# thygate/stable-diffusion-webui-depthmap-script

Measured on AMD Instinct MI355X. Metric: depth+stereo pairs/sec @1024x1024, higher is better.
Workload: dtype f16 (network) / f64 (stereo, normal map); 1 GPU; BASELINE config c3: MiDaS 3.1 DPT BEiT-L/16 512 forward (fp16, random-init weights seed 0, net 512x512, 1025 tokens) + depth->u16 + create_stereoimages(polylines_sharp, left-right, divergence 2.5%) + create_normalmap (Sobel 3) on 32 x 1024x1024 RGB per GPU, inputs resident in HBM; depth_network=dpt_beit_large_512, height=1024, width=1024, forward_launch=eager, library_convolutions=MIOpen, heuristic solver choice, overlap=single stream, parallelism=units sharded over 1 GPU(s), no data-path collective

## Files before the change

### include/depthstereo.h

```cpp
#ifndef DEPTHSTEREO_H
#define DEPTHSTEREO_H

#include <stddef.h>
#include <stdint.h>

#ifdef __cplusplus
extern "C" {
#endif

#define DS_VERSION 100

#define DS_OK            0
#define DS_EINVAL       -1
#define DS_EUNSUPPORTED -2
#define DS_EHIP         -3
#define DS_ENOMEM       -4

#define DS_DEPTH_U16 0
#define DS_DEPTH_F32 1
#define DS_DEPTH_F64 2

#define DS_FILL_NONE                0
#define DS_FILL_NAIVE               1
#define DS_FILL_NAIVE_INTERPOLATING 2
// ... 102 lines not shown
#define DS_PIX_U8  0
#define DS_PIX_U16 1
#define DS_PIX_I32 2
#define DS_PIX_F32 3

int ds_resize_lanczos(ds_ctx *ctx, const void *src, int pix, int n, int in_h, int in_w, int64_t src_px_stride, int64_t src_row_stride,
                      int64_t src_img_stride, void *dst, int out_h, int out_w, const int32_t *h_bounds, const void *h_coeffs, int h_taps,
                      const int32_t *v_bounds, const void *v_coeffs, int v_taps, void *tmp, void *stream);

#define DS_CD_WIDEN       0
#define DS_CD_SINGLE_BAND 1
#define DS_CD_MULTI_BAND  2
#define DS_CD_WORKSPACE_BLOCKS 256
int ds_custom_depth_to_f64(ds_ctx *ctx, const void *src, int pix, int n, int h, int w, int64_t src_px_stride, int64_t src_row_stride,
                           int64_t src_img_stride, int rule, double *out, double *workspace, void *stream);

#define DS_DTYPE_F16  1
#define DS_DTYPE_BF16 2
#define DS_DTYPE_F32  3

int ds_attention_fwd(ds_ctx *ctx, const void *qk, const void *vt, const void *bias_packed, void *out,
                     int B, int Np, int H, int n_valid, float scale, int dtype, void *stream);

int ds_attention_bias_pack(ds_ctx *ctx, const float *bias, int H, int n, int Np, int dtype, void *packed, void *stream);

int ds_attention_reload_env(void);

int ds_preprocess_bicubic(ds_ctx *ctx, const void *images, void *out, int batch, int in_h, int in_w, int out_h, int out_w,
                          int flip_channels, const float *mean, const float *std, int dtype, void *stream);

int ds_residual_layernorm(ds_ctx *ctx, const void *x, const void *branch, const void *gamma, const void *ln_weight,
                          const void *ln_bias, void *x_out, void *h_out, int64_t rows, int channels, float eps, int dtype,
                          void *stream);

int ds_reassemble_readout(ds_ctx *ctx, const void *proj, const void *clsvec, void *out, int batch, int tokens, int channels,
                          int dtype, void *stream);

int ds_bias_act_nhwc(ds_ctx *ctx, const void *x, const void *bias, const void *res1, const void *res2, void *out,
                     int64_t elements, int channels, int relu, int dtype, void *stream);

int ds_group_norm_nchw(ds_ctx *ctx, const void *x, const void *gamma, const void *beta, const void *res, void *out, int n, int channels,
                       int hw, int groups, float eps, int relu, int dtype, void *stream);

int ds_linear(ds_ctx *ctx, const void *x, const void *w, const void *bias, void *y, int64_t rows, int64_t out_features,
              int64_t in_features, int64_t ldy, int act, int dtype, void *stream);

int ds_linear_residual(ds_ctx *ctx, const void *x, const void *w, const void *bias, const void *gamma, const void *res, void *y,
                       int64_t rows, int64_t out_features, int64_t in_features, int dtype, void *stream);

int ds_linear_vt(ds_ctx *ctx, const void *w_v, const void *h, void *vt, int64_t channels, int64_t batch, int64_t tokens,
                 int64_t in_features, int dtype, void *stream);

int ds_linear_qkv(ds_ctx *ctx, const void *h, const void *w_qk, const void *b_qk, const void *w_v, void *qk, void *vt,
                  int64_t batch, int64_t tokens, int64_t qk_features, int64_t v_channels, int64_t in_features, int dtype, void *stream);

int ds_linear_shuffle(ds_ctx *ctx, const void *x, const void *w, const void *bias, void *y, int64_t pixels, int64_t in_features,
                      int width, int stride, int out_channels, int dtype, void *stream);

int ds_linear_readout(ds_ctx *ctx, const void *x, const void *w_tok, const void *cls_vec, void *y, int64_t images,
                      int64_t tokens_padded, int64_t tokens, int64_t out_features, int64_t in_features, int dtype, void *stream);

int ds_conv3x3_nhwc_pair(ds_ctx *ctx, const void *x0, const void *w0, void *y0, int batch0, int height0, int width0,
                         const void *x1, const void *w1, void *y1, int batch1, int height1, int width1,
                         int in_channels, int out_channels, int dtype, void *stream);

typedef struct ds_rows_problem {
    const void *x;
    int64_t x_row_pitch;
    const void *w;
    const void *bias;
    void *y;
} ds_rows_problem;
int ds_linear_rows4(ds_ctx *ctx, const ds_rows_problem *problems, int count, int64_t rows, int64_t out_features,
                    int64_t in_features, int dtype, void *stream);

int ds_row_stats(ds_ctx *ctx, const void *x, void *stats, int64_t rows, int channels, float eps, int dtype, void *stream);
int ds_linear_ln(ds_ctx *ctx, const void *x, const void *w_scaled, const float *colsum, const void *bias, const void *stats, void *y,
                 int64_t rows, int64_t out_features, int64_t in_features, int64_t ldy, int act, int dtype, void *stream);
int ds_linear_vt_ln(ds_ctx *ctx, const void *w_v_scaled, const float *colsum, const void *x, const void *stats, void *vt,
                    int64_t channels, int64_t batch, int64_t tokens, int64_t in_features, int dtype, void *stream);

int ds_linear_reload_env(void);

int ds_conv3x3_nhwc(ds_ctx *ctx, const void *x, const void *w, const void *bias, const void *res1, const void *res2, void *y,
                    int batch, int height, int width, int in_channels, int out_channels, int act, int dtype, void *stream);

int ds_conv3x3_nhwc_circular(ds_ctx *ctx, const void *x, const void *w, const void *bias, const void *res1, const void *res2, void *y,
                             int batch, int height, int width, int in_channels, int out_channels, int act, int dtype, void *stream);

int ds_upsample_bilinear_nhwc(ds_ctx *ctx, const void *in, void *out, int batch, int channels, int in_h, int in_w,
                              int out_h, int out_w, int align_corners, int dtype, void *stream);

int ds_dpt_head_front(ds_ctx *ctx, const void *x, const void *w, const void *bias, void *out, int batch, int in_h, int in_w,
                      int out_h, int out_w, int in_channels, int out_channels, int dtype, void *stream);

int ds_dpt_head_tail(ds_ctx *ctx, const void *x, int batch, int in_h, int in_w, int out_h, int out_w,
                     const void *conv3_wfrag, const float *conv3_bias, const float *conv1_weight, float conv1_bias,
                     int relu_out, void *out, int dtype, void *stream);

int ds_dpt_head_tail_circular(ds_ctx *ctx, const void *x, int batch, int in_h, int in_w, int out_h, int out_w,
                              const void *conv3_wfrag, const float *conv3_bias, const float *conv1_weight, float conv1_bias,
                              int relu_out, void *out, int dtype, void *stream);

int ds_gconv3x3_nhwc_f32(ds_ctx *ctx, const float *x, const float *w_gtio, const float *bias, float *y, int batch, int height, int width,
                         int channels, int channels_per_group, int relu, void *stream);
int ds_add_relu_f32(ds_ctx *ctx, const float *a, const float *b, float *y, int64_t count, void *stream);

int ds_bias_act_f32(ds_ctx *ctx, const float *x, const float *bias, const float *res, float *y, int64_t pixels, int channels, int relu,
                    void *stream);

int ds_dwconv_nhwc(ds_ctx *ctx, const void *x, const float *w, const float *bias_in, const float *bias, void *y, int batch, int in_h,
                   int in_w, int channels, int out_h, int out_w, int kernel, int stride, int pad_top, int pad_left, int dtype, void *stream);
int ds_relu_cat_f32(ds_ctx *ctx, const float *a, const float *b, float *y, int batch, int64_t plane, int channels_a, int channels_b, int layout,
                    void *stream);

int ds_boost_blend(ds_ctx *ctx, float *dst, int64_t dst_row_stride, int height, int width, const void *patches,
                   int n_patches, const float *preds, int pred_size, const float *mask_template, int mask_size,
                   void *stream);

int ds_preprocess_bicubic_rows(ds_ctx *ctx, const void *images, void *rows, int batch, int in_h, int in_w, int out_h, int out_w,
                               int flip_channels, const float *mean, const float *std, int patch, int n_pad, int kpad, int dtype,
                               void *stream);

int ds_tokens_fixup(ds_ctx *ctx, void *tokens, const void *cls, int batch, int n_pad, int n_valid, int channels, int dtype, void *stream);

int ds_upsample_bicubic_to_f32(ds_ctx *ctx, const void *in, void *out, int batch, int in_h, int in_w, int out_h, int out_w, int dtype,
                               void *stream);

int ds_im2col3x3_s2_nhwc(ds_ctx *ctx, const void *x, void *rows, int batch, int height, int width, int channels, int circular, int dtype,
                         void *stream);

#ifdef __cplusplus
}
#endif
#endif
```

### stable-diffusion-webui-depthmap-script_amd/csrc/ds_linear.hip

```cpp
#include "ds_common.h"

#include <stdlib.h>
#include <atomic>
#include <type_traits>

typedef _Float16 lf16x8 __attribute__((ext_vector_type(8)));
typedef __bf16 lbf16x8 __attribute__((ext_vector_type(8)));
typedef _Float16 lf16x4 __attribute__((ext_vector_type(4)));
typedef __bf16 lbf16x4 __attribute__((ext_vector_type(4)));
typedef float lf32x16 __attribute__((ext_vector_type(16)));
typedef float lf32x4 __attribute__((ext_vector_type(4)));

#if defined(DS_EXPERIMENTS) && defined(DS_LIN_MFMA32)
#define LN_MF16 0
#else
#define LN_MF16 1
#endif

#define LN_THREADS 512
#define LN_LDS_BYTES 131072
#define LN_HALF 16384
#define LN_B_BASE 65536

template <int BF16> struct ln_traits;
// ... 1087 lines not shown
    const int row0 = 32 * rb, col0 = cbk * 64, rows = P.rows;
    const int K = P.K, nst = K >> 7;
    const unsigned rowbytes = (unsigned)K * (unsigned)sizeof(T);
    const unsigned pitch = (unsigned)pk->pitch[prob];
    unsigned srcA, srcB[2];
    {
        const int j = 8 * (wid & 3) + (lane >> 3);
        const int jr = min(row0 + j, rows - 1) - row0;
        srcA = (unsigned)jr * pitch + (unsigned)(((lane & 7) ^ ((j >> 1) & 7)) << 4) + (unsigned)(wid >> 2) * 128u;
    }
#pragma unroll
    for (int i = 0; i < 2; ++i) {
        const int j = 8 * ((2 * wid + i) & 7) + (lane >> 3);
        srcB[i] = (unsigned)j * rowbytes + (unsigned)(((lane & 7) ^ ((j >> 1) & 7)) << 4) + (unsigned)(wid >> 2) * 128u;
    }
    const unsigned char *xb = (const unsigned char *)pk->x[prob] + (size_t)row0 * pitch;
    const unsigned char *wb = (const unsigned char *)pk->w[prob] + (size_t)col0 * rowbytes;
    const unsigned lds0 = (unsigned)(size_t)(__attribute__((address_space(3))) void *)lds;
    const bool mw = wid < 2;
    unsigned offA[8], offB[8];
#pragma unroll
    for (int u = 0; u < 8; ++u) {
        const int j = u >> 2, ks = u & 3;
        const unsigned sl = (unsigned)((LN_MF16 ? 4 * (ks >> 1) + (lane >> 4) : 2 * ks + hi) ^ ((lane >> 1) & 7)) << 4;
        const int lrow = LN_MF16 ? 16 * (ks & 1) + (lane & 15) : l31;
        offA[u] = (unsigned)j * 4096u + (unsigned)lrow * 128u + sl;
        offB[u] = 8192u + (unsigned)j * 8192u + (unsigned)((wid & 1) * 32 + lrow) * 128u + sl;
    }
    LN_SMALL_ACC(mine);
    const int e_row = row0 + LN_SMALL_ROW;
    const int e_cb = col0 + (wid & 1) * 32 + LN_SMALL_COL;
    const T *bias = (const T *)pk->bias[prob];
    V8 e_bv[2];
    if (mw && bias) {
#pragma unroll
        for (int k = 0; k < 2; ++k) e_bv[k] = *(const V8 *)(bias + e_cb + LN_SMALL_DCOL(k));
    }
#pragma unroll
    for (int t = 0; t < S - 1; ++t) TH_STAGE(t);
    V8 fa0[8], fb0[8], fa1[8], fb1[8];
    LN_WAIT_VM(12);
    LN_BARRIER();
    if (mw) {
        TH_READ(fa0, fb0, 0);
        __builtin_amdgcn_sched_barrier(0);
        LN_WAIT_LGKM0();
        __builtin_amdgcn_sched_barrier(0);
    }
    int st = 0;
    for (; st + 1 < nst; st += 2) {
        TH_STEP(fa0, fb0, fa1, fb1, st);
        TH_STEP(fa1, fb1, fa0, fb0, st + 1);
    }
    if (st < nst) TH_STEP(fa0, fb0, fa1, fb1, st);
    LN_WAIT_VM(0);
    if (!mw) return;

    T *yb = (T *)pk->y[prob];
#pragma unroll
    for (int k = 0; k < 2; ++k) {
        const int row = e_row + LN_SMALL_DROW(k), col = e_cb + LN_SMALL_DCOL(k);
        V8 bv;
        if (bias) bv = e_bv[k];
        else {
#pragma unroll
            for (int t = 0; t < 8; ++t) bv[t] = (T)0.f;
        }
        float v[8];
        LN_SMALL_V(v, mine, k);
        V8 o;
#pragma unroll
        for (int t = 0; t < 8; t += 2) {
            const lf32x2 u = {v[t] + (float)bv[t], v[t + 1] + (float)bv[t + 1]};
            o[t] = (T)u[0];
            o[t + 1] = (T)u[1];
        }
        if (row < rows) *(V8 *)(yb + (size_t)row * P.N + col) = o;
    }
}
#undef TH_STEP
#undef TH_READ
#undef TH_STAGE

struct LinOptions { int early, grid, ragged, ragged_den, ragged_ring, ragged_ksplit, ragged_ksplit_min, ragged_ksplit_keep, ragged_pipe, ragged_thin; };
static LinOptions g_lin_options;
static std::atomic<int> g_lin_options_state{0};
static void ln_read_options()
{
    auto geti = [](const char *name, int dflt) { const char *e = getenv(name); return e ? atoi(e) : dflt; };
    LinOptions o;
    o.early = geti("DS_LIN_EARLY", 1);
    o.grid = geti("DS_LIN_GRID", 0);
    o.ragged = geti("DS_LIN_RAGGED", 1);
    o.ragged_den = geti("DS_LIN_RAGGED_DEN", 4);
    o.ragged_ring = geti("DS_LIN_RAGGED_RING", 0);
    o.ragged_ksplit = geti("DS_LIN_RAGGED_KSPLIT", 1);
    o.ragged_ksplit_min = geti("DS_LIN_RAGGED_KSPLIT_MIN", 32);
    o.ragged_ksplit_keep = geti("DS_LIN_RAGGED_KSPLIT_KEEP", 8);
    if (o.ragged_ksplit_keep < 1) o.ragged_ksplit_keep = 1;
    o.ragged_pipe = geti("DS_LIN_RAGGED_PIPE", 1);
    o.ragged_thin = geti("DS_LIN_RAGGED_THIN", 1);
    g_lin_options = o;
    g_lin_options_state.store(1, std::memory_order_release);
}
static const LinOptions &ln_options()
{
    if (!g_lin_options_state.load(std::memory_order_acquire)) ln_read_options();
    return g_lin_options;
}
DS_API int ds_linear_reload_env(void)
{
    ln_read_options();
    return DS_OK;
}

#define LN_RG_COUNTER_BYTES 4096
#define LN_RG_MAX_WG 1024
static int ln_ragged_workspace(ds_ctx *ctx, int grid, hipStream_t stream)
{
    if (grid > LN_RG_MAX_WG) return 1;
    if (ctx->lin_ws && ctx->lin_ws_cleared == ctx->lin_ws) return DS_OK;
    hipStreamCaptureStatus cap = hipStreamCaptureStatusNone;
    if (hipStreamIsCapturing(stream, &cap) != hipSuccess || cap != hipStreamCaptureStatusNone) { (void)hipGetLastError(); return 1; }
    if (!ctx->lin_ws) {
        const int rc = ds_ctx_reserve(ctx, &ctx->lin_ws, &ctx->lin_ws_bytes, LN_RG_COUNTER_BYTES + (size_t)LN_RG_MAX_WG * 32768);
        if (rc != DS_OK) return rc;
    }
    DS_HIP_CHECK(hipMemsetAsync(ctx->lin_ws, 0, LN_RG_COUNTER_BYTES, stream));
    DS_HIP_CHECK(hipStreamSynchronize(stream));
    ctx->lin_ws_cleared = ctx->lin_ws;
    return DS_OK;
}

static int ln_ksplit_arch_ok(ds_ctx *ctx)
{
    static std::atomic<uint64_t> checked{0}, ok{0};
    const uint64_t bit = 1ull << (ctx->device & 63);
    if (!(checked.load(std::memory_order_acquire) & bit)) {
        hipDeviceProp_t prop;
        bool good = false;
        if (hipGetDeviceProperties(&prop, ctx->device) == hipSuccess)
            good = strncmp(prop.gcnArchName, "gfx950", 6) == 0 || strncmp(prop.gcnArchName, "gfx942", 6) == 0;
        else (void)hipGetLastError();
        if (good) ok.fetch_or(bit, std::memory_order_relaxed);
        checked.fetch_or(bit, std::memory_order_release);
    }
    return (ok.load(std::memory_order_relaxed) & bit) != 0;
}

template <int BF16, int EPI, int CONV, int RES, int VT = 0, int NH = 0>
static int ln_launch(ds_ctx *ctx, const LinParams &P0, hipStream_t stream)
{
    static std::atomic<uint64_t> attr_done{0};
    auto fn = k_linear256<BF16, EPI, CONV, RES, VT, NH>;
    DS_HIP_CHECK(hipSetDevice(ctx->device));
    const uint64_t bit = 1ull << (ctx->device & 63);
    if (!(attr_done.load(std::memory_order_relaxed) & bit)) {
        DS_HIP_CHECK(hipFuncSetAttribute((const void *)fn, hipFuncAttributeMaxDynamicSharedMemorySize, LN_LDS_BYTES));
        if constexpr (CONV == 0) {
            DS_HIP_CHECK(hipFuncSetAttribute((const void *)k_linear_ragged<BF16, EPI, RES, VT, 3>, hipFuncAttributeMaxDynamicSharedMemorySize, 3 * RG_SLOT));
            DS_HIP_CHECK(hipFuncSetAttribute((const void *)k_linear_ragged<BF16, EPI, RES, VT, 6>, hipFuncAttributeMaxDynamicSharedMemorySize, 6 * RG_SLOT));
            DS_HIP_CHECK(hipFuncSetAttribute((const void *)k_linear_ragged<BF16, EPI, RES, VT, 6, 1>, hipFuncAttributeMaxDynamicSharedMemorySize, 6 * RG_SLOT));
            if constexpr (VT == 0 && RES <= 1)
                DS_HIP_CHECK(hipFuncSetAttribute((const void *)k_linear_thin<BF16, EPI, RES>, hipFuncAttributeMaxDynamicSharedMemorySize, 6 * RG_SLOT));
        }
        attr_done.fetch_or(bit, std::memory_order_relaxed);
    }
    if (!ctx->ncu) {
        int ncu = 0;
        DS_HIP_CHECK(hipDeviceGetAttribute(&ncu, hipDeviceAttributeMultiprocessorCount, ctx->device));
        ctx->ncu = ncu >= 8 ? ncu / 8 * 8 : 8;
    }
    const LinOptions &O = ln_options();
    int grid = ctx->ncu;
    if (O.grid >= 8) grid = O.grid / 8 * 8;
    LinParams P = P0;
    P.bnw = NH ? 128 : 256;
    P.early = O.early;
#ifdef DS_EXPERIMENTS
    if (P.ablate) P.early = 0;
#endif
    const int ntiles = P.nbm * P.nbn;
    int ragged = 0;
    if (CONV == 0 && ntiles > grid) {
        const int r = ntiles % grid;
        if (O.ragged && r > 0 && O.ragged_den > 0 && O.ragged_den * r <= grid) ragged = r;
    }
    P.n_main = ntiles - ragged;
    const int deep = O.ragged_ring ? O.ragged_ring == 6 : 8 * ragged <= grid;
    bool thin = false;
    int th_nrb = 0;
    if constexpr (CONV == 0 && VT == 0 && RES <= 1) {
        th_nrb = (P.M - (P.nbm - 1) * 256 + 31) / 32;
        thin = O.ragged_thin && ragged > 0 && ragged == P.nbn && P.nbm >= 2 && (P.nbm - 1) % 8 == 0 && P.K % 128 == 0 && P.N % 64 == 0 &&
               O.ragged_ksplit <= 1 && th_nrb * (P.N / 64) <= ctx->ncu;
    }
    P.th_nrb = th_nrb;
    int ksl = 0;
    if (CONV == 0 && ragged && !thin && deep && 8 * ragged * (int)sizeof(int) <= LN_RG_COUNTER_BYTES && ln_ksplit_arch_ok(ctx)) {
        const int nt = P.K / 64;
        while (nt >= O.ragged_ksplit_min && (2 << ksl) <= O.ragged_ksplit && 8 * ragged * (2 << ksl) <= grid && nt % (2 << ksl) == 0 &&
               nt / (2 << ksl) >= O.ragged_ksplit_keep) ++ksl;
    }
    if (ksl > 0) {
        const int rc = ln_ragged_workspace(ctx, grid, stream);
        if (rc == DS_OK) { P.rg_cnt = (int *)ctx->lin_ws; P.rg_ws = (float *)((char *)ctx->lin_ws + LN_RG_COUNTER_BYTES); }
        else if (rc == 1) ksl = 0;
        else return rc;
    }
    P.rg_ksl = ksl;
    const int kt0 = ds_kt_begin(ctx, P.kt_kind, stream);
    hipLaunchKernelGGL(fn, dim3(P.n_main < grid ? P.n_main : grid), dim3(LN_THREADS), LN_LDS_BYTES, stream, P);
    ds_kt_end(ctx, P.kt_kind, kt0, stream);
    if constexpr (CONV == 0) {
        const int kt1 = ragged ? ds_kt_begin(ctx, P.kt_kind + DS_KT_RAGGED, stream) : -1;
        if (thin) {
            if constexpr (VT == 0 && RES <= 1) hipLaunchKernelGGL((k_linear_thin<BF16, EPI, RES>), dim3(th_nrb * (P.N / 64)), dim3(LN_THREADS), 6 * RG_SLOT, stream, P);
        } else if (ragged && deep && O.ragged_pipe) hipLaunchKernelGGL((k_linear_ragged<BF16, EPI, RES, VT, 6, 1>), dim3((8 * ragged) << ksl), dim3(LN_THREADS), 6 * RG_SLOT, stream, P);
        else if (ragged && deep) hipLaunchKernelGGL((k_linear_ragged<BF16, EPI, RES, VT, 6>), dim3((8 * ragged) << ksl), dim3(LN_THREADS), 6 * RG_SLOT, stream, P);
        else if (ragged) hipLaunchKernelGGL((k_linear_ragged<BF16, EPI, RES, VT, 3>), dim3(8 * ragged), dim3(LN_THREADS), 3 * RG_SLOT, stream, P);
        ds_kt_end(ctx, P.kt_kind + DS_KT_RAGGED, kt1, stream);
    }
    DS_HIP_CHECK(hipGetLastError());
    return DS_OK;
}

template <int BF16>
static int ln_launch_qkv(ds_ctx *ctx, const LinParams &PQ, const LinParams &PV0, hipStream_t stream)
{
    static std::atomic<uint64_t> attr_done{0};
    auto fn = k_linear256<BF16, 0, 0, 0, 4>;
    DS_HIP_CHECK(hipSetDevice(ctx->device));
    const uint64_t bit = 1ull << (ctx->device & 63);
    if (!(attr_done.load(std::memory_order_relaxed) & bit)) {
        DS_HIP_CHECK(hipFuncSetAttribute((const void *)fn, hipFuncAttributeMaxDynamicSharedMemorySize, LN_LDS_BYTES));
        DS_HIP_CHECK(hipFuncSetAttribute((const void *)k_linear_ragged<BF16, 0, 0, 1, 3>, hipFuncAttributeMaxDynamicSharedMemorySize, 3 * RG_SLOT));
        DS_HIP_CHECK(hipFuncSetAttribute((const void *)k_linear_ragged<BF16, 0, 0, 1, 6>, hipFuncAttributeMaxDynamicSharedMemorySize, 6 * RG_SLOT));
        DS_HIP_CHECK(hipFuncSetAttribute((const void *)k_linear_ragged<BF16, 0, 0, 1, 6, 1>, hipFuncAttributeMaxDynamicSharedMemorySize, 6 * RG_SLOT));
        attr_done.fetch_or(bit, std::memory_order_relaxed);
    }
    if (!ctx->ncu) {
        int ncu = 0;
        DS_HIP_CHECK(hipDeviceGetAttribute(&ncu, hipDeviceAttributeMultiprocessorCount, ctx->device));
        ctx->ncu = ncu >= 8 ? ncu / 8 * 8 : 8;
    }
    const LinOptions &O = ln_options();
    int grid = ctx->ncu;
    if (O.grid >= 8) grid = O.grid / 8 * 8;
    const int t0 = PQ.nbm * PQ.nbn, t1 = PV0.nbm * PV0.nbn, ntiles = t0 + t1;
    int ragged = 0;
    if (ntiles > grid) {
        const int r = ntiles % grid;
        if (O.ragged && r > 0 && O.ragged_den > 0 && O.ragged_den * r <= grid && r <= t1) ragged = r;
    }
    LinParams P = PQ, PV = PV0;
    P.bnw = PV.bnw = 256;
    P.early = O.early;
    P.x1 = PV.x; P.w1 = PV.w; P.y1 = PV.y;
    P.seg_t0 = t0; P.M1 = PV.M; P.nbm1 = PV.nbm; P.nbn1 = PV.nbn;
    P.vt_np = PV.vt_np; P.vt_c = PV.vt_c; P.vt_magic = PV.vt_magic;
    P.n_main = ntiles - ragged;
    PV.n_main = t1 - ragged;
    const int kt0 = ds_kt_begin(ctx, DS_KT_LINEAR, stream);
    hipLaunchKernelGGL(fn, dim3(P.n_main < grid ? P.n_main : grid), dim3(LN_THREADS), LN_LDS_BYTES, stream, P);
    ds_kt_end(ctx, DS_KT_LINEAR, kt0, stream);
    if (ragged) {
        const int deep = O.ragged_ring ? O.ragged_ring == 6 : 8 * ragged <= grid;
        const int kt1 = ds_kt_begin(ctx, DS_KT_LINEAR + DS_KT_RAGGED, stream);
        if (deep && O.ragged_pipe) hipLaunchKernelGGL((k_linear_ragged<BF16, 0, 0, 1, 6, 1>), dim3(8 * ragged), dim3(LN_THREADS), 6 * RG_SLOT, stream, PV);
        else if (deep) hipLaunchKernelGGL((k_linear_ragged<BF16, 0, 0, 1, 6>), dim3(8 * ragged), dim3(LN_THREADS), 6 * RG_SLOT, stream, PV);
        else hipLaunchKernelGGL((k_linear_ragged<BF16, 0, 0, 1, 3>), dim3(8 * ragged), dim3(LN_THREADS), 3 * RG_SLOT, stream, PV);
        ds_kt_end(ctx, DS_KT_LINEAR + DS_KT_RAGGED, kt1, stream);
    }
    DS_HIP_CHECK(hipGetLastError());
    return DS_OK;
}

template <int BF16>
static int ln_dispatch_dense(ds_ctx *ctx, const LinParams &P, int act, hipStream_t st)
{
    if (act == 1) return ln_launch<BF16, 1, 0, 0>(ctx, P, st);
    if (act == 2) return ln_launch<BF16, 2, 0, 0>(ctx, P, st);
    return ln_launch<BF16, 0, 0, 0>(ctx, P, st);
}

template <int BF16, int CIRC>
static int ln_dispatch_conv(ds_ctx *ctx, const LinParams &P, int act, hipStream_t st)
{
    constexpr int CV = CIRC ? 3 : 1, CVR = CIRC ? 4 : 2;
    const int res = P.res1 ? (P.res2 ? 2 : 1) : 0;
    if (act & 4) {
        if (P.N % 256 == 0 && (act & 3) == 2 && res == 0) return ln_launch<BF16, 2, CVR, 0>(ctx, P, st);
        ds_set_error("ds_conv3x3_nhwc[_circular]: act 4 (ReLU on x) is built for act 2 | 4 without residual operands and out_channels %% 256 == 0");
        return DS_EUNSUPPORTED;
    }
    if (P.N % 256 != 0) {
        if (act == 2) return ln_launch<BF16, 2, CV, 0, 0, 1>(ctx, P, st);
        return ln_launch<BF16, 0, CV, 0, 0, 1>(ctx, P, st);
    }
    if (act == 2) {
        if (res == 2) return ln_launch<BF16, 2, CV, 2>(ctx, P, st);
        if (res == 1) return ln_launch<BF16, 2, CV, 1>(ctx, P, st);
        return ln_launch<BF16, 2, CV, 0>(ctx, P, st);
    }
    if (res == 2) return ln_launch<BF16, 0, CV, 2>(ctx, P, st);
    if (res == 1) return ln_launch<BF16, 0, CV, 1>(ctx, P, st);
    return ln_launch<BF16, 0, CV, 0>(ctx, P, st);
}

DS_API int ds_linear(ds_ctx *ctx, const void *x, const void *w, const void *bias, void *y, int64_t rows, int64_t out_features,
                     int64_t in_features, int64_t ldy, int act, int dtype, void *stream)
{
    DS_REQUIRE(ctx && x && w && y, DS_EINVAL, "ds_linear: null argument");
    DS_REQUIRE(rows >= 256 && rows < (1ll << 31) - 256, DS_EINVAL, "ds_linear: rows must be >= 256 (one tile)");
    DS_REQUIRE(out_features > 0 && out_features % 256 == 0, DS_EINVAL, "ds_linear: out_features must be a multiple of 256");
    DS_REQUIRE(in_features >= 128 && in_features % 128 == 0 && in_features <= 16384, DS_EINVAL,
               "ds_linear: in_features must be a multiple of 128 (<= 16384)");
    DS_REQUIRE(ldy >= out_features && ldy % 8 == 0, DS_EINVAL, "ds_linear: ldy must be >= out_features and a multiple of 8");
    DS_REQUIRE(((uintptr_t)x & 15) == 0 && ((uintptr_t)w & 15) == 0 && ((uintptr_t)y & 15) == 0 && (!bias || ((uintptr_t)bias & 15) == 0), DS_EINVAL,
               "ds_linear: x, w (the LDS-DMA sources), y and bias must be 16-byte aligned");
    DS_REQUIRE(act >= 0 && act <= 2, DS_EINVAL, "ds_linear: act must be 0 (none), 1 (erf-GELU) or 2 (ReLU)");
    DS_REQUIRE(dtype == DS_DTYPE_F16 || dtype == DS_DTYPE_BF16, DS_EINVAL, "ds_linear: dtype must be f16 or bf16");
    LinParams P;
    memset(&P, 0, sizeof(P));
    P.x = x; P.w = w; P.bias = bias; P.y = y;
    P.M = (int)rows; P.N = (int)out_features; P.K = (int)in_features;
    P.nbm = (int)((rows + 255) / 256); P.nbn = (int)(out_features / 256);
    P.ldy = ldy;
    P.kt_kind = act == 1 ? DS_KT_LINEAR_GELU : DS_KT_LINEAR;
#ifdef DS_EXPERIMENTS
    P.ablate = getenv("DS_LIN_ABLATE") ? atoi(getenv("DS_LIN_ABLATE")) : 0;
    P.stagger = getenv("DS_LIN_STAGGER_US") ? (int)(atof(getenv("DS_LIN_STAGGER_US")) * 100.0) : 0;
#endif
    return dtype == DS_DTYPE_F16 ? ln_dispatch_dense<0>(ctx, P, act, (hipStream_t)stream) : ln_dispatch_dense<1>(ctx, P, act, (hipStream_t)stream);
}

DS_API int ds_linear_residual(ds_ctx *ctx, const void *x, const void *w, const void *bias, const void *gamma, const void *res, void *y,
                              int64_t rows, int64_t out_features, int64_t in_features, int dtype, void *stream)
{
    DS_REQUIRE(ctx && x && w && y && res, DS_EINVAL, "ds_linear_residual: null argument");
    DS_REQUIRE(rows >= 256 && rows < (1ll << 31) - 256, DS_EINVAL, "ds_linear_residual: rows must be >= 256 (one tile)");
    DS_REQUIRE(out_features > 0 && out_features % 256 == 0, DS_EINVAL, "ds_linear_residual: out_features must be a multiple of 256");
    DS_REQUIRE(in_features >= 128 && in_features % 128 == 0 && in_features <= 16384, DS_EINVAL,
               "ds_linear_residual: in_features must be a multiple of 128 (<= 16384)");
    DS_REQUIRE(dtype == DS_DTYPE_F16 || dtype == DS_DTYPE_BF16, DS_EINVAL, "ds_linear_residual: dtype must be f16 or bf16");
    DS_REQUIRE(((uintptr_t)x & 15) == 0 && ((uintptr_t)w & 15) == 0 && ((uintptr_t)y & 15) == 0 && ((uintptr_t)res & 15) == 0 &&
               ((uintptr_t)bias & 15) == 0 && ((uintptr_t)gamma & 15) == 0 && y != res,
               DS_EINVAL, "ds_linear_residual: x, w, y, res, bias and gamma must be 16-byte aligned, and y must not alias res");
    LinParams P;
    memset(&P, 0, sizeof(P));
    P.x = x; P.w = w; P.bias = bias; P.gamma = gamma; P.res1 = res; P.y = y;
    P.M = (int)rows; P.N = (int)out_features; P.K = (int)in_features;
    P.nbm = (int)((rows + 255) / 256); P.nbn = (int)(out_features / 256);
    P.ldy = out_features;
    P.kt_kind = DS_KT_LINEAR_RESIDUAL;
// ... 343 lines not shown
```

### stable-diffusion-webui-depthmap-script_amd/src/_native.py

```python
import collections
import ctypes
import math
import os
import threading

import numpy as np

_PKG_ROOT = os.path.dirname(os.path.dirname(os.path.abspath(__file__)))
LIB_PATH = os.environ.get("DS_NATIVE_LIB") or os.path.join(_PKG_ROOT, "libdepthstereo_hip.so")

DS_DEPTH_U16, DS_DEPTH_F32, DS_DEPTH_F64 = 0, 1, 2
FILL_IDS = {"none": 0, "naive": 1, "naive_interpolating": 2, "polylines_soft": 3, "polylines_sharp": 4}

EXPORTS = [
    "ds_version", "ds_last_error", "ds_normalmap_f64", "ds_normalmap_gradient_f32", "ds_reassemble_readout", "ds_bias_act_nhwc", "ds_linear", "ds_linear_residual", "ds_linear_vt", "ds_linear_qkv", "ds_conv3x3_nhwc", "ds_ctx_create", "ds_ctx_destroy", "ds_stereo_warp", "ds_depth_minmax",
    "ds_stereo_last_exact_rows", "ds_copy_view", "ds_overlap_red_cyan", "ds_normalmap", "ds_depth_to_u16",
    "ds_convert_to_i16", "ds_profile_enable", "ds_profile_last_ms", "ds_stereo_last_stats", "ds_attention_fwd", "ds_attention_bias_pack", "ds_colorize_u16", "ds_residual_layernorm", "ds_boost_blend", "ds_upsample_bilinear_nhwc", "ds_dpt_head_tail", "ds_preprocess_bicubic", "ds_linear_reload_env", "ds_attention_reload_env", "ds_normalmap_selfcheck", "ds_normalmap_gradient_f16", "ds_normalmap_gradient_blur_f32",
    "ds_linear_shuffle", "ds_linear_readout", "ds_linear_rows4", "ds_conv3x3_nhwc_pair", "ds_kernel_timer_enable", "ds_kernel_timer_read", "ds_kernel_timer_read_each", "ds_group_norm_nchw",
    "ds_row_stats", "ds_linear_ln", "ds_linear_vt_ln", "ds_gconv3x3_nhwc_f32", "ds_add_relu_f32", "ds_bias_act_f32", "ds_relu_cat_f32",
    "ds_dwconv_nhwc", "ds_resize_lanczos", "ds_custom_depth_to_f64", "ds_conv3x3_nhwc_circular", "ds_dpt_head_tail_circular",
    "ds_normalmap_wrap", "ds_normalmap_f64_wrap", "ds_normalmap_gradient_f32_wrap", "ds_normalmap_gradient_f16_wrap", "ds_normalmap_gradient_blur_f32_wrap",
    "ds_bilateral_u16", "ds_joint_bilateral_u16", "ds_frame_luma_hist", "ds_temporal_smooth5_f32", "ds_temporal_joint_bilateral_u16",
    "ds_preprocess_bicubic_rows", "ds_tokens_fixup", "ds_upsample_bicubic_to_f32", "ds_im2col3x3_s2_nhwc", "ds_dpt_head_front",
]


class DepthStereoError(RuntimeError):
    pass


class ds_rows_problem(ctypes.Structure):
    _fields_ = [("x", ctypes.c_void_p), ("x_row_pitch", ctypes.c_int64), ("w", ctypes.c_void_p), ("bias", ctypes.c_void_p),
                ("y", ctypes.c_void_p)]


class ds_eye(ctypes.Structure):
    _fields_ = [("divergence_px", ctypes.c_double), ("separation_px", ctypes.c_double),
                ("out", ctypes.c_void_p), ("out_row_stride", ctypes.c_int64), ("out_img_stride", ctypes.c_int64)]


_lib = None
_lib_lock = threading.Lock()

CALLS = collections.Counter()


def lib():
    global _lib
    with _lib_lock:
        if _lib is None:
            if not os.path.exists(LIB_PATH):
                raise DepthStereoError(
                    f"{LIB_PATH} is missing: build it with `python __graft_entry__.py build` "
                    "(hipcc --offload-arch=gfx950).  There is no CPU fallback.")
            L = ctypes.CDLL(LIB_PATH)
            vp, ci, cd, i64 = ctypes.c_void_p, ctypes.c_int, ctypes.c_double, ctypes.c_int64
            L.ds_version.restype = ci
            L.ds_last_error.restype = ctypes.c_char_p
            L.ds_ctx_create.argtypes = [ctypes.POINTER(vp), ci]
            L.ds_ctx_destroy.argtypes = [vp]
            L.ds_stereo_warp.argtypes = [vp, vp, vp, ci, ci, ci, ci, ci, cd, vp, ci, ctypes.POINTER(ds_eye), ci, vp]
            L.ds_depth_minmax.argtypes = [vp, vp, ci, ci, ci, ci, vp, vp]
            L.ds_stereo_last_exact_rows.argtypes = [vp, ctypes.POINTER(i64), vp]
            L.ds_copy_view.argtypes = [vp, vp, i64, i64, vp, i64, i64, ci, ci, i64, vp]
            L.ds_overlap_red_cyan.argtypes = [vp, vp, i64, i64, vp, i64, i64, ci, ci, ci, ci, vp, vp]
            L.ds_normalmap.argtypes = [vp, vp, ci, ci, ci, ci, ci, ci, ci, vp, vp]
            L.ds_normalmap_f64.argtypes = [vp, vp, ci, ci, ci, ci, ci, ci, ci, vp, vp]
            L.ds_normalmap_gradient_f32.argtypes = [vp, vp, ci, ci, ci, ci, vp, vp]
            L.ds_normalmap_gradient_f16.argtypes = [vp, vp, ci, ci, ci, ci, vp, vp]
            L.ds_normalmap_gradient_blur_f32.argtypes = [vp, vp, ci, ci, ci, ci, ci, ci, vp, vp]
            for name in ("ds_normalmap", "ds_normalmap_f64", "ds_normalmap_gradient_f32", "ds_normalmap_gradient_f16", "ds_normalmap_gradient_blur_f32"):
                getattr(L, name + "_wrap").argtypes = getattr(L, name).argtypes
            L.ds_bilateral_u16.argtypes = [vp, vp, ci, ci, ci, ci, vp, vp, ci, vp, vp]
            L.ds_joint_bilateral_u16.argtypes = [vp, vp, vp, ci, ci, ci, ci, ci, vp, vp, ci, vp, vp]
            L.ds_frame_luma_hist.argtypes = [vp, vp, ci, ci, ci, ci, vp, vp]
            L.ds_temporal_smooth5_f32.argtypes = [vp, vp, ci, i64, ci, ci, ci, ci, vp, vp]
            L.ds_temporal_joint_bilateral_u16.argtypes = [vp, vp, vp, ci, ci, ci, ci, ci, vp, vp, ci, ci, ci, ci, vp, vp]
            L.ds_depth_to_u16.argtypes = [vp, vp, ci, ci, ci, ci, vp, vp, vp]
            L.ds_convert_to_i16.argtypes = [vp, vp, ci, i64, vp, vp]
            L.ds_stereo_last_stats.argtypes = [vp, ctypes.POINTER(i64), vp]
            L.ds_attention_fwd.argtypes = [vp, vp, vp, vp, vp, ci, ci, ci, ci, ctypes.c_float, ci, vp]
            L.ds_normalmap_selfcheck.argtypes = [vp, ctypes.c_ulonglong, ctypes.c_ulonglong, ctypes.c_ulonglong, ctypes.POINTER(ctypes.c_ulonglong), vp]
            L.ds_attention_bias_pack.argtypes = [vp, vp, ci, ci, ci, ci, vp, vp]
            L.ds_colorize_u16.argtypes = [vp, vp, ci, ci, ci, vp, vp, ci, vp, vp]
            L.ds_residual_layernorm.argtypes = [vp, vp, vp, vp, vp, vp, vp, vp, i64, ci, ctypes.c_float, ci, vp]
            L.ds_boost_blend.argtypes = [vp, vp, i64, ci, ci, vp, ci, vp, ci, vp, ci, vp]
            L.ds_upsample_bilinear_nhwc.argtypes = [vp, vp, vp, ci, ci, ci, ci, ci, ci, ci, ci, vp]
            L.ds_dpt_head_tail.argtypes = [vp, vp, ci, ci, ci, ci, ci, vp, vp, vp, ctypes.c_float, ci, vp, ci, vp]
            L.ds_dpt_head_tail_circular.argtypes = L.ds_dpt_head_tail.argtypes
            L.ds_dpt_head_front.argtypes = [vp, vp, vp, vp, vp, ci, ci, ci, ci, ci, ci, ci, ci, vp]
            L.ds_preprocess_bicubic.argtypes = [vp, vp, vp, ci, ci, ci, ci, ci, ci, ctypes.POINTER(ctypes.c_float),
                                                ctypes.POINTER(ctypes.c_float), ci, vp]
            L.ds_preprocess_bicubic_rows.argtypes = [vp, vp, vp, ci, ci, ci, ci, ci, ci, ctypes.POINTER(ctypes.c_float),
                                                     ctypes.POINTER(ctypes.c_float), ci, ci, ci, ci, vp]
            L.ds_tokens_fixup.argtypes = [vp, vp, vp, ci, ci, ci, ci, ci, vp]
            L.ds_upsample_bicubic_to_f32.argtypes = [vp, vp, vp, ci, ci, ci, ci, ci, ci, vp]
            L.ds_im2col3x3_s2_nhwc.argtypes = [vp, vp, vp, ci, ci, ci, ci, ci, ci, vp]
            L.ds_reassemble_readout.argtypes = [vp, vp, vp, vp, ci, ci, ci, ci, vp]
            L.ds_bias_act_nhwc.argtypes = [vp, vp, vp, vp, vp, vp, i64, ci, ci, ci, vp]
            L.ds_group_norm_nchw.argtypes = [vp, vp, vp, vp, vp, vp, ci, ci, ci, ci, ctypes.c_float, ci, ci, vp]
# ... 512 lines not shown
    def dtype(self):
        return self.data.dtype


def attention_bias_pack(bias, npad, dtype):
    torch = require_gpu()
    npad = (int(npad) + 63) // 64 * 64
    assert bias.is_cuda and bias.dim() == 3 and bias.shape[1] == bias.shape[2] and dtype in (torch.float16, torch.bfloat16)
    h, n = int(bias.shape[0]), int(bias.shape[1])
    src = bias.detach().float().contiguous()
    out = torch.empty((h * npad * npad,), dtype=dtype, device=bias.device)
    CALLS["ds_attention_bias_pack"] += 1
    _check(lib().ds_attention_bias_pack(ctx_for(_dev_index(src)), src.data_ptr(), h, n, int(npad),
                                        1 if dtype == torch.float16 else 2, out.data_ptr(), _stream(src)))
    return PackedAttentionBias(out, h, n, int(npad))


def attention_fwd(qk, vt, n_valid, scale, bias=None):
    torch = require_gpu()
    assert qk.is_cuda and vt.is_cuda and qk.dtype == vt.dtype and qk.dtype in (torch.float16, torch.bfloat16)
    b, npad, two, h, d = qk.shape
    assert two == 2 and d == 64 and npad % 8 == 0 and tuple(vt.shape) == (b, h * 64, npad), (qk.shape, vt.shape)
    qk = qk.contiguous()
    vt = vt.contiguous()
    if bias is not None:
        assert isinstance(bias, PackedAttentionBias), "bias must come from attention_bias_pack"
        assert (bias.heads, bias.npad, bias.dtype) == (h, (npad + 63) // 64 * 64, qk.dtype) and bias.data.device == qk.device
    out = torch.empty((b, npad, h * 64), dtype=qk.dtype, device=qk.device)
    dt = 1 if qk.dtype == torch.float16 else 2
    CALLS["ds_attention_fwd"] += 1
    _check(lib().ds_attention_fwd(ctx_for(_dev_index(qk)), qk.data_ptr(), vt.data_ptr(),
                                  bias.data.data_ptr() if bias is not None else None, out.data_ptr(),
                                  b, npad, h, int(n_valid), float(scale), dt, _stream(qk)))
    return out


def residual_layernorm(x, branch, gamma, ln_weight, ln_bias, eps=1e-6):
    torch = require_gpu()
    assert x.is_cuda and x.dtype in (torch.float16, torch.bfloat16)
    x = x.contiguous()
    c = x.shape[-1]
    rows = x.numel() // c
    h = torch.empty_like(x)
    dt = 1 if x.dtype == torch.float16 else 2
    if branch is None:
        x_out, bp = x, None
    else:
        branch = branch.contiguous()
        assert branch.shape == x.shape and branch.dtype == x.dtype
        x_out = torch.empty_like(x)
        bp = branch.data_ptr()
    g = None if gamma is None else gamma.to(x.dtype).contiguous()
    w, b = ln_weight.to(x.dtype).contiguous(), ln_bias.to(x.dtype).contiguous()
    CALLS["ds_residual_layernorm"] += 1
    _check(lib().ds_residual_layernorm(ctx_for(_dev_index(x)), x.data_ptr(), bp, None if g is None else g.data_ptr(),
                                       w.data_ptr(), b.data_ptr(), None if branch is None else x_out.data_ptr(), h.data_ptr(),
                                       rows, c, float(eps), dt, _stream(x)))
    return x_out, h


def reassemble_readout(proj, clsvec):
    torch = require_gpu()
    assert proj.is_cuda and proj.dtype in (torch.float16, torch.bfloat16) and proj.dim() == 3 and clsvec.dtype == proj.dtype
    b, n, c = proj.shape
    proj, clsvec = proj.contiguous(), clsvec.contiguous()
    assert tuple(clsvec.shape) == (b, c)
    out = torch.empty((b, n - 1, c), dtype=proj.dtype, device=proj.device)
    CALLS["ds_reassemble_readout"] += 1
    _check(lib().ds_reassemble_readout(ctx_for(_dev_index(proj)), proj.data_ptr(), clsvec.data_ptr(), out.data_ptr(), b, n, c,
                                       1 if proj.dtype == torch.float16 else 2, _stream(proj)))
    return out


def linear_env(**switches):
    for k, v in switches.items():
        assert k.startswith("DS_LIN_")
        if v is None:
            os.environ.pop(k, None)
        else:
            os.environ[k] = str(v)
    _check(lib().ds_linear_reload_env())


def normalmap_selfcheck(k0, stride, count):
    torch = require_gpu()
    bad = ctypes.c_ulonglong(0)
    _check(lib().ds_normalmap_selfcheck(ctx_for(torch.cuda.current_device()), ctypes.c_ulonglong(k0), ctypes.c_ulonglong(stride),
                                        ctypes.c_ulonglong(count), ctypes.byref(bad), None))
    return int(bad.value)


def attention_env(**switches):
    for k, v in switches.items():
        assert k.startswith("DS_ATT_")
        if v is None:
            os.environ.pop(k, None)
        else:
            os.environ[k] = str(v)
    _check(lib().ds_attention_reload_env())


def linear_supported(x, weight):
    return weight.shape[0] % 256 == 0 and weight.shape[1] % 128 == 0 and 128 <= weight.shape[1] <= 16384 and x.numel() > 0


def linear(x, weight, bias=None, gelu=False):
    torch = require_gpu()
    assert x.is_cuda and x.dtype in (torch.float16, torch.bfloat16) and linear_supported(x, weight)
    k = x.shape[-1]
    n = weight.shape[0]
    assert weight.shape[1] == k
    x2 = x.reshape(-1, k)
    if not x2.is_contiguous():
        x2 = x2.contiguous()
    rows = x2.shape[0]
    if rows < 256:
        x2 = torch.cat([x2, x2.new_zeros((256 - rows, k))])
    w = weight.detach()
    w = w if (w.dtype == x.dtype and w.is_contiguous()) else w.to(x.dtype).contiguous()
    b = None
    if bias is not None:
        b = bias.detach()
        b = b if (b.dtype == x.dtype and b.is_contiguous()) else b.to(x.dtype).contiguous()
    out = torch.empty((x2.shape[0], n), dtype=x.dtype, device=x.device)
    CALLS["ds_linear"] += 1
    _check(lib().ds_linear(ctx_for(_dev_index(x)), x2.data_ptr(), w.data_ptr(), None if b is None else b.data_ptr(),
                           out.data_ptr(), x2.shape[0], n, k, n, 1 if gelu else 0,
                           1 if x.dtype == torch.float16 else 2, _stream(x)))
    return out[:rows].view(x.shape[:-1] + (n,))


def linear_residual(x, weight, bias, gamma, residual):
    torch = require_gpu()
    assert x.is_cuda and x.dtype in (torch.float16, torch.bfloat16) and linear_supported(x, weight)
    k, n = x.shape[-1], weight.shape[0]
    x2 = x.reshape(-1, k).contiguous()
    r2 = residual.reshape(-1, n).contiguous()
    assert x2.shape[0] == r2.shape[0] >= 256 and r2.dtype == x.dtype

    def prep(t):
        if t is None:
            return None
        t = t.detach()
        return t if (t.dtype == x.dtype and t.is_contiguous()) else t.to(x.dtype).contiguous()
    w, b, g = prep(weight), prep(bias), prep(gamma)
    out = torch.empty_like(r2)
    CALLS["ds_linear_residual"] += 1
    _check(lib().ds_linear_residual(ctx_for(_dev_index(x)), x2.data_ptr(), w.data_ptr(), None if b is None else b.data_ptr(),
                                    None if g is None else g.data_ptr(), r2.data_ptr(), out.data_ptr(), x2.shape[0], n, k,
                                    1 if x.dtype == torch.float16 else 2, _stream(x)))
    return out.view(residual.shape)


def linear_readout_supported(x_padded, w_tok):
    return (x_padded.dim() == 3 and x_padded.is_contiguous() and x_padded.shape[0] * x_padded.shape[1] >= 256
            and w_tok.shape[0] % 256 == 0 and w_tok.shape[1] == x_padded.shape[2] and x_padded.shape[2] % 128 == 0
            and 128 <= x_padded.shape[2] <= 16384 and x_padded.shape[0] * x_padded.shape[1] * x_padded.shape[1] < (1 << 32))


def linear_readout(x_padded, n_tokens, w_tok, cls_vec):
    torch = require_gpu()
    assert x_padded.is_cuda and x_padded.dtype in (torch.float16, torch.bfloat16) and linear_readout_supported(x_padded, w_tok)
    b, npad, k = x_padded.shape
    n = w_tok.shape[0]
    assert 2 <= n_tokens <= npad and tuple(cls_vec.shape) == (b, n)
    w = w_tok.detach()
# ... 573 lines not shown
```

Measured before the change: 943.1 pairs/s.

## Add 32-column thin ragged-tail linear kernel to spread tail work across more CUs

Adds k_linear_thin32, a variant of the thin ragged-tail GEMM kernel that tiles 32 rows by 32 columns instead of 64 columns. It uses a deeper 9-stage LDS ring and only two MFMA waves. It is chosen by default whenever the thin path applies and the doubled block count still fits the CU count, so the leftover-row GEMM runs on more workgroups. The trade is lower per-block arithmetic intensity and idle waves, in exchange for better CU occupancy on the ragged tail. It also adds route counters with an exported query function and a rounds option that relaxes the CU-count gate.

```diff
diff --git a/include/depthstereo.h b/include/depthstereo.h
--- a/include/depthstereo.h
+++ b/include/depthstereo.h
@@ -208,6 +208,8 @@
 
 int ds_linear_reload_env(void);
 
+int ds_linear_ragged_routes(int64_t counts[3]);
+
 int ds_conv3x3_nhwc(ds_ctx *ctx, const void *x, const void *w, const void *bias, const void *res1, const void *res2, void *y,
                     int batch, int height, int width, int in_channels, int out_channels, int act, int dtype, void *stream);
 
diff --git a/stable-diffusion-webui-depthmap-script_amd/csrc/ds_linear.hip b/stable-diffusion-webui-depthmap-script_amd/csrc/ds_linear.hip
--- a/stable-diffusion-webui-depthmap-script_amd/csrc/ds_linear.hip
+++ b/stable-diffusion-webui-depthmap-script_amd/csrc/ds_linear.hip
@@ -1193,7 +1193,141 @@
 #undef TH_READ
 #undef TH_STAGE
 
-struct LinOptions { int early, grid, ragged, ragged_den, ragged_ring, ragged_ksplit, ragged_ksplit_min, ragged_ksplit_keep, ragged_pipe, ragged_thin; };
+#if LN_MF16
+#define T32_SLOT 16384
+#define T32_S 9
+template <int BF16, int EPI, int RES>
+__global__ __launch_bounds__(LN_THREADS) void k_linear_thin32(LinParams P)
+{
+    typedef ln_traits<BF16> TR;
+    typedef typename TR::T T;
+    typedef typename TR::V8 V8;
+    constexpr int S = T32_S;
+    static_assert(S * T32_SLOT == 6 * RG_SLOT, "the ring fills the 144 KB of k_linear_thin");
+    extern __shared__ __attribute__((aligned(1024))) unsigned char lds[];
+    const int tid = threadIdx.x, lane = tid & 63;
+    const int wid = __builtin_amdgcn_readfirstlane(tid >> 6);
+    const int ncb = P.N >> 5;
+    const int rb = (int)blockIdx.x / ncb, cbk = (int)blockIdx.x - rb * ncb;
+    const int row0 = P.M - 32 * (P.th_nrb - rb), col0 = cbk * 32;
+    const int K = P.K, nst = K >> 7;
+    const unsigned rowbytes = (unsigned)K * (unsigned)sizeof(T);
+    unsigned src;
+    {
+        const int j = 8 * (wid & 3) + (lane >> 3);
+        src = (unsigned)j * rowbytes + (unsigned)(((lane & 7) ^ ((j >> 1) & 7)) << 4) + (unsigned)(wid >> 2) * 128u;
+    }
+    const unsigned char *xb = (const unsigned char *)P.x + (size_t)row0 * rowbytes;
+    const unsigned char *wb = (const unsigned char *)P.w + (size_t)col0 * rowbytes;
+    const unsigned lds0 = (unsigned)(size_t)(__attribute__((address_space(3))) void *)lds;
+#define T32_STAGE(st_)                                                                                                   \
+    do {                                                                                                                 \
+        const int sc_ = min((st_), nst - 1);                 \
+        const unsigned sl_ = lds0 + (unsigned)((st_) % S) * T32_SLOT;                                                     \
+        ln_dma_s(xb + (size_t)sc_ * 256, src, sl_ + (unsigned)wid * 1024u);                                               \
+        ln_dma_s(wb + (size_t)sc_ * 256, src, sl_ + 8192u + (unsigned)wid * 1024u);                                       \
+    } while (0)
+    const bool mw = wid < 2;
+    unsigned offA[4], offB[8];
+#pragma unroll
+    for (int u = 0; u < 4; ++u) {
+        const int j = u >> 1, ks = u & 1;
+        const unsigned sl = (unsigned)((4 * ks + (lane >> 4)) ^ ((lane >> 1) & 7)) << 4;
+        offA[u] = (unsigned)j * 4096u + (unsigned)(16 * (wid & 1) + (lane & 15)) * 128u + sl;
+#pragma unroll
+        for (int cb = 0; cb < 2; ++cb) offB[2 * u + cb] = 8192u + (unsigned)j * 4096u + (unsigned)(16 * cb + (lane & 15)) * 128u + sl;
+    }
+    lf32x4 acc[2];
+#pragma unroll
+    for (int r = 0; r < 8; ++r) acc[r >> 2][r & 3] = 0.f;
+    const int e_row = row0 + 16 * (wid & 1) + LN_SMALL_ROW;
+    const int e_col = col0 + LN_SMALL_COL;
+    V8 e_bv, e_gv, e_rv;
+    if (mw) {
+        if (P.bias) e_bv = *(const V8 *)((const T *)P.bias + e_col);
+        if (EPI == 3) e_gv = *(const V8 *)((const T *)P.gamma + e_col);
+        if (RES >= 1) e_rv = *(const V8 *)((const T *)P.res1 + (size_t)e_row * P.ldy + e_col);
+    }
+#pragma unroll
+    for (int t = 0; t < S - 1; ++t) T32_STAGE(t);
+    V8 fa0[4], fb0[8], fa1[4], fb1[8];
+#define T32_READ(fa_, fb_, st_)                                                                                          \
+    do {                                                                                                                 \
+        const unsigned char *sb_ = lds + ((st_) % S) * T32_SLOT;                                                         \
+        _Pragma("unroll") for (int u = 0; u < 4; ++u) fa_[u] = *(const V8 *)(sb_ + offA[u]);                             \
+        _Pragma("unroll") for (int u = 0; u < 8; ++u) fb_[u] = *(const V8 *)(sb_ + offB[u]);                             \
+    } while (0)
+#define T32_STEP(ca_, cb_, na_, nb_, st_)                                                                                \
+    do {                                                                                                                 \
+        LN_WAIT_VM(12);                                                                                                  \
+        LN_BARRIER();                                                                                                    \
+        T32_STAGE((st_) + S - 1);                                                                                        \
+        if (mw) {                                                                                                        \
+            T32_READ(na_, nb_, (st_) + 1);                                                                               \
+            __builtin_amdgcn_sched_barrier(0);                                                                           \
+            _Pragma("unroll") for (int u_ = 0; u_ < 4; ++u_) _Pragma("unroll") for (int c_ = 0; c_ < 2; ++c_)            \
+                acc[c_] = TR::mfma16(cb_[2 * u_ + c_], ca_[u_], acc[c_]);                                                \
+            __builtin_amdgcn_sched_barrier(0);                                                                           \
+            LN_WAIT_LGKM0();                                                                                             \
+            __builtin_amdgcn_sched_barrier(0);                                                                           \
+        }                                                                                                                \
+    } while (0)
+    LN_WAIT_VM(14);
+    LN_BARRIER();
+    if (mw) {
+        T32_READ(fa0, fb0, 0);
+        __builtin_amdgcn_sched_barrier(0);
+        LN_WAIT_LGKM0();
+        __builtin_amdgcn_sched_barrier(0);
+    }
+    int st = 0;
+    for (; st + 1 < nst; st += 2) {
+        T32_STEP(fa0, fb0, fa1, fb1, st);
+        T32_STEP(fa1, fb1, fa0, fb0, st + 1);
+    }
+    if (st < nst) T32_STEP(fa0, fb0, fa1, fb1, st);
+    LN_WAIT_VM(0);
+#undef T32_STEP
+#undef T32_READ
+#undef T32_STAGE
+    if (!mw) return;
+
+    V8 bv;
+    if (P.bias) bv = e_bv;
+    else {
+#pragma unroll
+        for (int t = 0; t < 8; ++t) bv[t] = (T)0.f;
+    }
+    float v[8];
+#pragma unroll
+    for (int t = 0; t < 4; ++t) {
+        const auto sw = __builtin_amdgcn_permlane16_swap(__float_as_uint(acc[0][t]), __float_as_uint(acc[1][t]), false, false);
+        v[t] = __uint_as_float(sw[0]);
+        v[4 + t] = __uint_as_float(sw[1]);
+    }
+    if (EPI == 4 || EPI == 5) {
+        const float2 stt = P.ln_stats[e_row];
+        const float4 s0 = *(const float4 *)(P.ln_colsum + e_col), s1 = *(const float4 *)(P.ln_colsum + e_col + 4);
+        const float sc[8] = {s0.x, s0.y, s0.z, s0.w, s1.x, s1.y, s1.z, s1.w};
+#pragma unroll
+        for (int t = 0; t < 8; ++t) v[t] = __builtin_fmaf(v[t], stt.x, stt.y * sc[t]);
+    }
+    V8 o;
+#pragma unroll
+    for (int t = 0; t < 8; t += 2) {
+        lf32x2 u = {v[t] + (float)bv[t], v[t + 1] + (float)bv[t + 1]};
+        if (EPI == 3) u *= (lf32x2){(float)e_gv[t], (float)e_gv[t + 1]};
+        if (RES >= 1) u += (lf32x2){(float)e_rv[t], (float)e_rv[t + 1]};
+        if (EPI == 1 || EPI == 5) u = ln_gelu2(u);
+        if (EPI == 2) u = (lf32x2){fmaxf(u[0], 0.f), fmaxf(u[1], 0.f)};
+        o[t] = (T)u[0];
+        o[t + 1] = (T)u[1];
+    }
+    *(V8 *)((T *)P.y + (size_t)e_row * P.ldy + e_col) = o;
+}
+#endif
+
+struct LinOptions { int early, grid, ragged, ragged_den, ragged_ring, ragged_ksplit, ragged_ksplit_min, ragged_ksplit_keep, ragged_pipe, ragged_thin, ragged_thin_cols, ragged_thin_rounds; };
 static LinOptions g_lin_options;
 static std::atomic<int> g_lin_options_state{0};
 static void ln_read_options()
@@ -1211,6 +1345,9 @@
     if (o.ragged_ksplit_keep < 1) o.ragged_ksplit_keep = 1;
     o.ragged_pipe = geti("DS_LIN_RAGGED_PIPE", 1);
     o.ragged_thin = geti("DS_LIN_RAGGED_THIN", 1);
+    o.ragged_thin_cols = geti("DS_LIN_RAGGED_THIN_COLS", -1);
+    o.ragged_thin_rounds = geti("DS_LIN_RAGGED_THIN_ROUNDS", 1);
+    if (o.ragged_thin_rounds < 1) o.ragged_thin_rounds = 1;
     g_lin_options = o;
     g_lin_options_state.store(1, std::memory_order_release);
 }
@@ -1222,6 +1359,14 @@
 DS_API int ds_linear_reload_env(void)
 {
     ln_read_options();
+    return DS_OK;
+}
+
+enum { LN_ROUTE_RAGGED = 0, LN_ROUTE_THIN = 1, LN_ROUTE_THIN32 = 2 };
+static std::atomic<long long> g_lin_ragged_routes[3];
+DS_API int ds_linear_ragged_routes(int64_t counts[3])
+{
+    for (int i = 0; i < 3; ++i) counts[i] = g_lin_ragged_routes[i].load(std::memory_order_relaxed);
     return DS_OK;
 }
 
@@ -1273,7 +1418,12 @@
             DS_HIP_CHECK(hipFuncSetAttribute((const void *)k_linear_ragged<BF16, EPI, RES, VT, 6>, hipFuncAttributeMaxDynamicSharedMemorySize, 6 * RG_SLOT));
             DS_HIP_CHECK(hipFuncSetAttribute((const void *)k_linear_ragged<BF16, EPI, RES, VT, 6, 1>, hipFuncAttributeMaxDynamicSharedMemorySize, 6 * RG_SLOT));
             if constexpr (VT == 0 && RES <= 1)
+            {
                 DS_HIP_CHECK(hipFuncSetAttribute((const void *)k_linear_thin<BF16, EPI, RES>, hipFuncAttributeMaxDynamicSharedMemorySize, 6 * RG_SLOT));
+#if LN_MF16
+                DS_HIP_CHECK(hipFuncSetAttribute((const void *)k_linear_thin32<BF16, EPI, RES>, hipFuncAttributeMaxDynamicSharedMemorySize, T32_S * T32_SLOT));
+#endif
+            }
         }
         attr_done.fetch_or(bit, std::memory_order_relaxed);
     }
@@ -1304,9 +1454,13 @@
     if constexpr (CONV == 0 && VT == 0 && RES <= 1) {
         th_nrb = (P.M - (P.nbm - 1) * 256 + 31) / 32;
         thin = O.ragged_thin && ragged > 0 && ragged == P.nbn && P.nbm >= 2 && (P.nbm - 1) % 8 == 0 && P.K % 128 == 0 && P.N % 64 == 0 &&
-               O.ragged_ksplit <= 1 && th_nrb * (P.N / 64) <= ctx->ncu;
+               O.ragged_ksplit <= 1 && th_nrb * (P.N / 64) <= ctx->ncu * O.ragged_thin_rounds;
     }
     P.th_nrb = th_nrb;
+    bool thin32 = false;
+#if LN_MF16
+    if (thin && O.ragged_thin_cols != 0 && O.ragged_thin_cols != 64 && th_nrb * (P.N / 32) <= ctx->ncu * O.ragged_thin_rounds) thin32 = true;
+#endif
     int ksl = 0;
     if (CONV == 0 && ragged && !thin && deep && 8 * ragged * (int)sizeof(int) <= LN_RG_COUNTER_BYTES && ln_ksplit_arch_ok(ctx)) {
         const int nt = P.K / 64;
@@ -1325,12 +1479,17 @@
     ds_kt_end(ctx, P.kt_kind, kt0, stream);
     if constexpr (CONV == 0) {
         const int kt1 = ragged ? ds_kt_begin(ctx, P.kt_kind + DS_KT_RAGGED, stream) : -1;
-        if (thin) {
+        if (thin32) {
+#if LN_MF16
+            if constexpr (VT == 0 && RES <= 1) hipLaunchKernelGGL((k_linear_thin32<BF16, EPI, RES>), dim3(th_nrb * (P.N / 32)), dim3(LN_THREADS), T32_S * T32_SLOT, stream, P);
+#endif
+        } else if (thin) {
             if constexpr (VT == 0 && RES <= 1) hipLaunchKernelGGL((k_linear_thin<BF16, EPI, RES>), dim3(th_nrb * (P.N / 64)), dim3(LN_THREADS), 6 * RG_SLOT, stream, P);
         } else if (ragged && deep && O.ragged_pipe) hipLaunchKernelGGL((k_linear_ragged<BF16, EPI, RES, VT, 6, 1>), dim3((8 * ragged) << ksl), dim3(LN_THREADS), 6 * RG_SLOT, stream, P);
         else if (ragged && deep) hipLaunchKernelGGL((k_linear_ragged<BF16, EPI, RES, VT, 6>), dim3((8 * ragged) << ksl), dim3(LN_THREADS), 6 * RG_SLOT, stream, P);
         else if (ragged) hipLaunchKernelGGL((k_linear_ragged<BF16, EPI, RES, VT, 3>), dim3(8 * ragged), dim3(LN_THREADS), 3 * RG_SLOT, stream, P);
         ds_kt_end(ctx, P.kt_kind + DS_KT_RAGGED, kt1, stream);
+        if (ragged) g_lin_ragged_routes[thin32 ? LN_ROUTE_THIN32 : thin ? LN_ROUTE_THIN : LN_ROUTE_RAGGED].fetch_add(1, std::memory_order_relaxed);
     }
     DS_HIP_CHECK(hipGetLastError());
     return DS_OK;
@@ -1382,6 +1541,7 @@
         else if (deep) hipLaunchKernelGGL((k_linear_ragged<BF16, 0, 0, 1, 6>), dim3(8 * ragged), dim3(LN_THREADS), 6 * RG_SLOT, stream, PV);
         else hipLaunchKernelGGL((k_linear_ragged<BF16, 0, 0, 1, 3>), dim3(8 * ragged), dim3(LN_THREADS), 3 * RG_SLOT, stream, PV);
         ds_kt_end(ctx, DS_KT_LINEAR + DS_KT_RAGGED, kt1, stream);
+        g_lin_ragged_routes[LN_ROUTE_RAGGED].fetch_add(1, std::memory_order_relaxed);
     }
     DS_HIP_CHECK(hipGetLastError());
     return DS_OK;
diff --git a/stable-diffusion-webui-depthmap-script_amd/src/_native.py b/stable-diffusion-webui-depthmap-script_amd/src/_native.py
--- a/stable-diffusion-webui-depthmap-script_amd/src/_native.py
+++ b/stable-diffusion-webui-depthmap-script_amd/src/_native.py
@@ -15,7 +15,7 @@
 EXPORTS = [
     "ds_version", "ds_last_error", "ds_normalmap_f64", "ds_normalmap_gradient_f32", "ds_reassemble_readout", "ds_bias_act_nhwc", "ds_linear", "ds_linear_residual", "ds_linear_vt", "ds_linear_qkv", "ds_conv3x3_nhwc", "ds_ctx_create", "ds_ctx_destroy", "ds_stereo_warp", "ds_depth_minmax",
     "ds_stereo_last_exact_rows", "ds_copy_view", "ds_overlap_red_cyan", "ds_normalmap", "ds_depth_to_u16",
-    "ds_convert_to_i16", "ds_profile_enable", "ds_profile_last_ms", "ds_stereo_last_stats", "ds_attention_fwd", "ds_attention_bias_pack", "ds_colorize_u16", "ds_residual_layernorm", "ds_boost_blend", "ds_upsample_bilinear_nhwc", "ds_dpt_head_tail", "ds_preprocess_bicubic", "ds_linear_reload_env", "ds_attention_reload_env", "ds_normalmap_selfcheck", "ds_normalmap_gradient_f16", "ds_normalmap_gradient_blur_f32",
+    "ds_convert_to_i16", "ds_profile_enable", "ds_profile_last_ms", "ds_stereo_last_stats", "ds_attention_fwd", "ds_attention_bias_pack", "ds_colorize_u16", "ds_residual_layernorm", "ds_boost_blend", "ds_upsample_bilinear_nhwc", "ds_dpt_head_tail", "ds_preprocess_bicubic", "ds_linear_reload_env", "ds_linear_ragged_routes", "ds_attention_reload_env", "ds_normalmap_selfcheck", "ds_normalmap_gradient_f16", "ds_normalmap_gradient_blur_f32",
     "ds_linear_shuffle", "ds_linear_readout", "ds_linear_rows4", "ds_conv3x3_nhwc_pair", "ds_kernel_timer_enable", "ds_kernel_timer_read", "ds_kernel_timer_read_each", "ds_group_norm_nchw",
     "ds_row_stats", "ds_linear_ln", "ds_linear_vt_ln", "ds_gconv3x3_nhwc_f32", "ds_add_relu_f32", "ds_bias_act_f32", "ds_relu_cat_f32",
     "ds_dwconv_nhwc", "ds_resize_lanczos", "ds_custom_depth_to_f64", "ds_conv3x3_nhwc_circular", "ds_dpt_head_tail_circular",
@@ -694,6 +694,12 @@
     _check(lib().ds_linear_reload_env())
 
 
+def linear_ragged_routes():
+    c = (ctypes.c_int64 * 3)()
+    _check(lib().ds_linear_ragged_routes(c))
+    return {"ragged": int(c[0]), "thin": int(c[1]), "thin32": int(c[2])}
+
+
 def normalmap_selfcheck(k0, stride, count):
     torch = require_gpu()
     bad = ctypes.c_ulonglong(0)
```

Result: no change. 945.1 pairs/s, median of 6 (+0.2%).
